# facebookresearch/KeypointNeRF

Measured on AMD Instinct MI355X. Metric: rendered rays/sec (64 coarse + 64 fine samples/ray), higher is better.
Workload: dtype f32 (dominant kernel: every fp32 operand as two fp16 pieces (22 bits, the residual formed exactly), three fp16-MFMA products per term set (hh hl lh: all terms above 2^-24 relative), fp32 accumulation; everything else fp32)

## Files before the change

### include/kpnerf.h

```cpp
#ifndef KPNERF_H
#define KPNERF_H

#include <stddef.h>
#include <stdint.h>

#ifdef __cplusplus
extern "C" {
#endif

#define KPN_ABI_VERSION 10
#define KPN_N_KPT 24
#define KPN_MAX_VIEWS 16

enum { KPN_OK = 0, KPN_EINVAL = -1, KPN_ELAUNCH = -2, KPN_EWORKSPACE = -3 };

int kpn_abi_version(void);
const char* kpn_last_error(void);
int kpn_is_device_build(void);

size_t kpn_plain_weight_floats(void);
size_t kpn_packed_weight_floats(void);
int kpn_pack_weights(const float* plain_host, float* packed_host);
int kpn_pack_weights_device(const float* plain_dev, float* packed_dev, void* stream);

typedef struct kpn_scene_desc {
    int32_t n_views;
    int32_t src_h, src_w;
    int32_t geo0_h, geo0_w;
    int32_t geo1_h, geo1_w;
    int32_t tex_h, tex_w;
    int32_t disable_fg_mask;
    float znear, zfar;
    float nml_scale;
    float sigma;
    const float* KRT;
    const float* extrin;
    const float* kpt3d;
    const float* img;
    const uint8_t* fg_mask;
    const float* geo0;
    const float* geo1;
    const float* tex;
} kpn_scene_desc;

size_t kpn_scene_workspace_bytes(const kpn_scene_desc* desc);
int kpn_scene_prepare(const kpn_scene_desc* desc, void* scene_ws, void* stream);


int kpn_ray_bbox_intersection(const float* bounds, const float* orig, const float* direct, int64_t n_rays,
                              float* near_out, float* far_out, uint8_t* hit_out, void* stream);

int kpn_make_rays(const float* K, const float* RT, float znear, float zfar, const float* bounds, int32_t x0,
                  int32_t y0, int32_t step, int32_t nx, int32_t ny, float* dirs, float* cam_pos, float* near_out,
                  float* far_out, void* stream);

int kpn_importance_sample(const float* contrib, const float* z, const float* u, int64_t n_rays, int32_t d_minus_2,
                          int32_t n_samples, float* samples_out, void* stream);

int kpn_rgba2out(const float* rgba, const float* z, int64_t n_rays, int32_t n_samples, float* color, float* depth,
                 float* alpha, float* contrib, float* sdf, void* stream);

int kpn_rgba2out_backward(const float* rgba, const float* z, int64_t n_rays, int32_t n_samples, const float* d_color,
                          const float* d_depth, const float* d_alpha, const float* d_sdf, float* d_rgba, void* stream);

size_t kpn_geo_rows_backward_workspace_bytes(int64_t n_points, int32_t n_views);
int kpn_geo_rows_backward(const kpn_scene_desc* desc, const void* scene_ws, const float* packed_weights, int64_t n_points,
                          const float* pts, uint32_t keep_mask, const float* d_x, float* d_plain, float* d_geo0,
                          float* d_geo1, void* workspace, size_t workspace_bytes, void* stream);

size_t kpn_query_backward_geometry_workspace_bytes(int64_t n_points, int32_t n_views);
int kpn_query_backward_geometry(const kpn_scene_desc* desc, const void* scene_ws, const float* packed_weights,
                                int64_t n_points, const float* pts, int32_t mode, uint32_t keep_mask, const float* noise,
                                float noise_std, const float* d_out, float* d_plain, float* d_geo0, float* d_geo1,
                                void* workspace, size_t workspace_bytes, void* stream);

size_t kpn_query_backward_workspace_bytes(int64_t n_points, int32_t n_views);
int kpn_query_backward(const kpn_scene_desc* desc, const void* scene_ws, const float* packed_weights, int64_t n_points,
                       const float* pts, const float* view, int32_t mode, uint32_t keep_mask, const float* noise,
                       float noise_std, const float* d_out, float* d_plain, float* d_geo0, float* d_geo1, float* d_tex,
// ... 223 lines not shown
```

### keypointnerf_amd/csrc/api_render.hip

```cpp
namespace {
struct RenderLayout { size_t cam_pos, dirs, nearv, farv, zc, zf, zn, src, rgba, rgba_c, rgba_n, contrib, color, depth, alpha, sdf, query, total; int64_t chunk; };
int64_t pick_chunk(const kpn_scene_desc* d, const kpn_render_args* a) {
    const int64_t R = (int64_t)a->nx * a->ny;
    int64_t c = a->chunk_rays;
    if (c <= 0) {
        const int64_t cmax = 262144;
        const int64_t npass = (R + cmax - 1) / cmax;
        c = ((R + npass - 1) / npass + 63) / 64 * 64;
    }
    return c < R ? c : R;
}
RenderLayout render_layout(const kpn_scene_desc* d, const kpn_render_args* a) {
    RenderLayout L;
    const int64_t R = (int64_t)a->nx * a->ny;
    const int64_t C = pick_chunk(d, a);
    const int64_t Sfull = a->n_coarse + (a->fine ? a->n_fine : 0);
    Carver c;
    L.chunk = C;
    L.cam_pos = c.take(64);
    L.dirs = c.take((size_t)R * 3 * 4);
    L.nearv = c.take((size_t)R * 4);
    L.farv = c.take((size_t)R * 4);
    L.zc = c.take((size_t)C * a->n_coarse * 4);
    L.zf = c.take((size_t)C * Sfull * 4);
// ... 38 lines not shown
}

__global__ void k_store_planar(int64_t r0, int64_t n, int64_t R, int C, const float* __restrict__ src, float* __restrict__ dst) {
    const int64_t i = (int64_t)blockIdx.x * blockDim.x + threadIdx.x;
    if (i >= n * C) return;
    const int64_t r = i / C;
    const int c = (int)(i - r * C);
    dst[(int64_t)c * R + r0 + r] = src[i];
}
__global__ void k_load_planar(int64_t r0, int64_t n, int64_t R, int C, const float* __restrict__ src, float* __restrict__ dst) {
    const int64_t i = (int64_t)blockIdx.x * blockDim.x + threadIdx.x;
    if (i >= n * C) return;
    const int64_t r = i / C;
    const int c = (int)(i - r * C);
    dst[i] = src ? src[(int64_t)c * R + r0 + r] : 0.0f;
}
struct PlanarChunk {
    void* stream; int64_t r0, n, R;
    void store(float* dst, const float* src, int C) const {
        if (dst) KPN_LAUNCH(k_store_planar, grid1d(n * C, 256), dim3(256), stream, r0, n, R, C, src, dst);
    }
    void load(float* dst, const float* src, int C) const {
        KPN_LAUNCH(k_load_planar, grid1d(n * C, 256), dim3(256), stream, r0, n, R, C, src, dst);
    }
};

extern "C" size_t kpn_render_workspace_bytes(const kpn_scene_desc* d, const kpn_render_args* a) {
    if (check_desc(d) != KPN_OK || check_render(a) != KPN_OK) return 0;
    return render_layout(d, a).total;
}

static void launch_fine_samples(void* stream, int64_t n, int Sc, int Sf, const float* zc, const float* contrib,
                                const float* u, float* zf, float* znew, int16_t* src) {
    const dim3 grid((unsigned)(n + 3 < 4 * 8192 ? (n + 3) / 4 : 8192));
    if (Sc <= 64 && Sf <= 64)
        KPN_LAUNCH(k_fine_samples_w<true>, grid, dim3(256), stream, n, Sc, Sf, zc, contrib, u, zf, znew, src);
    else
        KPN_LAUNCH(k_fine_samples_w<false>, grid, dim3(256), stream, n, Sc, Sf, zc, contrib, u, zf, znew, src);
}

static int render_impl(const kpn_scene_desc* d, const void* scene_ws, const float* wp, const kpn_render_args* a,
                       const kpn_train_args* t, void* ws, size_t ws_bytes, void* stream) {
    if (int e = check_desc(d)) return e;
    if (int e = check_render(a)) return e;
    KPN_REQUIRE(scene_ws && wp && ws, "null pointer");
    if (t) if (int e = check_train(d, a, t, false)) return e;
    const RenderLayout L = render_layout(d, a);
    if (ws_bytes < L.total) return fail(KPN_EWORKSPACE, "render workspace too small");
    char* base = static_cast<char*>(ws);
    auto F = [&](size_t off) { return reinterpret_cast<float*>(base + off); };
    kpn_scene_dev sc = scene_dev(d, scene_ws);
    const int64_t R = (int64_t)a->nx * a->ny;
    const int Sc = a->n_coarse, Sf = a->fine ? a->n_fine : 0, Sfull = Sc + Sf;
    KPN_LAUNCH(k_make_rays, grid1d(R, 256), dim3(256), stream, a->K, a->RT, a->znear, a->zfar, a->bounds, (int)a->x0, (int)a->y0,
               (int)a->step, (int)(a->step_y > 0 ? a->step_y : a->step), (int)a->nx, (int)a->ny, t ? (const int*)t->pix : (const int*)nullptr, F(L.dirs), F(L.cam_pos),
               F(L.nearv), F(L.farv));
    for (int64_t r0 = 0; r0 < R; r0 += L.chunk) {
        const int64_t n = (R - r0) < L.chunk ? (R - r0) : L.chunk;
        const float* dirs = F(L.dirs) + r0 * 3;
        const PlanarChunk pl{stream, r0, n, R};
        KPN_LAUNCH(k_coarse_z, grid1d(n * Sc, 256), dim3(256), stream, n, Sc, (const float*)(F(L.nearv) + r0),
                   (const float*)(F(L.farv) + r0), t ? t->u_coarse + r0 * Sc : (const float*)nullptr, F(L.zc));
        kpn_points ps{nullptr, nullptr, F(L.cam_pos), dirs, F(L.zc), Sc,
                      (t && t->rand_noise_std != 0.0f) ? t->noise_coarse + r0 * Sc : nullptr, t ? t->rand_noise_std : 0.0f};
        sc.keep = t ? t->keep_coarse : 0xFFFFFFFFu;
        const char* nr = getenv("KPN_NO_COARSE_REUSE");
        const bool no_reuse = nr && atoi(nr);
        const bool reuse = (t == nullptr) && a->fine && !no_reuse;
// ... 235 lines not shown
```

### keypointnerf_amd/csrc/api_scene.hip

```cpp
namespace {
struct SceneLayout { size_t table, rgbm, geo0, geo1, tex, flags, total; };
SceneLayout scene_layout(const kpn_scene_desc* d) {
    SceneLayout L;
    Carver c;
    L.table = c.take((size_t)d->n_views * KPN_TBL_STRIDE, 64);
    L.rgbm = c.take((size_t)d->n_views * d->src_h * d->src_w * 4, 64);
    L.geo0 = c.take((size_t)d->n_views * d->geo0_h * d->geo0_w * 64, 64);
    L.geo1 = c.take((size_t)d->n_views * d->geo1_h * d->geo1_w * 8, 64);
    L.tex = c.take((size_t)d->n_views * d->tex_h * d->tex_w * 8, 64);
    L.flags = c.take((size_t)KPN_SCENE_FLAG_FLOATS, 64);
    L.total = c.o;
    return L;
}
int check_desc(const kpn_scene_desc* d) {
    KPN_REQUIRE(d != nullptr, "scene desc is null");
    KPN_REQUIRE(d->n_views >= 1 && d->n_views <= KPN_MAX_VIEWS, "n_views out of range");
    KPN_REQUIRE(d->src_h > 1 && d->src_w > 1 && d->geo0_h > 1 && d->geo0_w > 1 && d->geo1_h > 1 && d->geo1_w > 1 &&
                d->tex_h > 1 && d->tex_w > 1, "map sizes must be > 1");
    KPN_REQUIRE(d->zfar > d->znear && d->nml_scale > 0.0f && d->sigma > 0.0f, "bad scalar parameters");
    KPN_REQUIRE(d->KRT && d->extrin && d->kpt3d && d->img && d->geo0 && d->geo1 && d->tex, "null scene tensor");
    KPN_REQUIRE(d->disable_fg_mask || d->fg_mask, "fg_mask is null");
    return KPN_OK;
}
kpn_scene_dev scene_dev(const kpn_scene_desc* d, const void* ws) {
    const SceneLayout L = scene_layout(d);
    const float* base = static_cast<const float*>(ws);
    kpn_scene_dev s;
    s.V = d->n_views; s.H = d->src_h; s.W = d->src_w;
    s.g0h = d->geo0_h; s.g0w = d->geo0_w; s.g1h = d->geo1_h; s.g1w = d->geo1_w; s.th = d->tex_h; s.tw = d->tex_w;
    s.disable_fg_mask = d->disable_fg_mask;
    s.znear = d->znear; s.zfar = d->zfar; s.nml_scale = d->nml_scale;
    s.two_sigma2 = (float)(2.0 * ((double)d->sigma * (double)d->sigma));
    s.keep = 0xFFFFFFFFu;
    s.table = base + L.table; s.rgbm = base + L.rgbm; s.geo0 = base + L.geo0; s.geo1 = base + L.geo1; s.tex = base + L.tex;
    s.flags = base + L.flags;
    return s;
}
}

extern "C" size_t kpn_scene_workspace_bytes(const kpn_scene_desc* d) {
    if (check_desc(d) != KPN_OK) return 0;
    return scene_layout(d).total * sizeof(float);
}

extern "C" int kpn_scene_prepare(const kpn_scene_desc* d, void* scene_ws, void* stream) {
    if (int e = check_desc(d)) return e;
    KPN_REQUIRE(scene_ws != nullptr, "scene workspace is null");
    const SceneLayout L = scene_layout(d);
    float* base = static_cast<float*>(scene_ws);
    const int V = d->n_views;
    float* flags = base + L.flags;
    KPN_LAUNCH(k_scene_table, dim3(1), dim3(64), stream, V, d->KRT, d->extrin, d->kpt3d, base + L.table, flags);
    const int64_t HW = (int64_t)d->src_h * d->src_w;
    KPN_LAUNCH(k_pack_rgbm, grid1d(V * HW, 256), dim3(256), stream, (int64_t)(V * HW), HW, d->img,
               d->disable_fg_mask ? (const uint8_t*)nullptr : d->fg_mask, base + L.rgbm, flags);
    const int64_t hw0 = (int64_t)d->geo0_h * d->geo0_w, hw1 = (int64_t)d->geo1_h * d->geo1_w, hwt = (int64_t)d->tex_h * d->tex_w;
    KPN_LAUNCH(k_nchw_to_nhwc, grid1d(V * hw0 * 64, 256), dim3(256), stream, (int64_t)(V * hw0 * 64), 64, hw0, d->geo0, base + L.geo0, flags);
    KPN_LAUNCH(k_nchw_to_nhwc, grid1d(V * hw1 * 8, 256), dim3(256), stream, (int64_t)(V * hw1 * 8), 8, hw1, d->geo1, base + L.geo1, flags);
    KPN_LAUNCH(k_nchw_to_nhwc, grid1d(V * hwt * 8, 256), dim3(256), stream, (int64_t)(V * hwt * 8), 8, hwt, d->tex, base + L.tex, flags);
    return check_launch("kpn_scene_prepare");
}

extern "C" int kpn_ray_bbox_intersection(const float* bounds, const float* orig, const float* direct, int64_t R,
                                         float* near_o, float* far_o, uint8_t* hit_o, void* stream) {
    KPN_REQUIRE(bounds && orig && direct && near_o && far_o && hit_o, "null pointer");
    KPN_REQUIRE(R >= 0, "negative ray count");
    if (R == 0) return KPN_OK;
    KPN_LAUNCH(k_ray_bbox, grid1d(R, 256), dim3(256), stream, R, bounds, orig, direct, near_o, far_o, hit_o);
    return check_launch("kpn_ray_bbox_intersection");
}

extern "C" int kpn_make_rays(const float* K, const float* RT, float znear, float zfar, const float* bounds, int32_t x0,
                             int32_t y0, int32_t step, int32_t nx, int32_t ny, float* dirs, float* cam_pos,
                             float* near_o, float* far_o, void* stream) {
    KPN_REQUIRE(K && RT && bounds && dirs && cam_pos && near_o && far_o, "null pointer");
    KPN_REQUIRE(nx > 0 && ny > 0 && step > 0, "bad pixel grid");
    KPN_LAUNCH(k_make_rays, grid1d((int64_t)nx * ny, 256), dim3(256), stream, K, RT, znear, zfar, bounds, (int)x0, (int)y0,
               (int)step, (int)step, (int)nx, (int)ny, (const int*)nullptr, dirs, cam_pos, near_o, far_o);
    return check_launch("kpn_make_rays");
}

extern "C" int kpn_importance_sample(const float* contrib, const float* z, const float* u, int64_t R, int32_t Dm2,
                                     int32_t n, float* out, void* stream) {
    KPN_REQUIRE(contrib && z && out, "null pointer");
    KPN_REQUIRE(Dm2 >= 1 && Dm2 + 1 <= KPN_IS_MAXD, "bin count out of range (<= 128)");
    KPN_REQUIRE(n >= 1 && R >= 0, "bad sizes");
    if (R == 0) return KPN_OK;
    KPN_LAUNCH(k_importance, grid1d(R, 64), dim3(64), stream, R, (int)Dm2, (int)n, contrib, z, u, out);
    return check_launch("kpn_importance_sample");
}

static void launch_rgba2out(void* stream, int64_t R, int S, const float* rgba, const float* z, float* color, float* depth,
// ... 39 lines not shown
```

### keypointnerf_amd/csrc/ray_kernels.hip

```cpp
#include "kpn_device.h"

__device__ __forceinline__ void kpn_note_absmax(float* __restrict__ flags, float a) {
    int u = __float_as_int(a) & 0x7fffffff;
#pragma unroll
    for (int o = 32; o > 0; o >>= 1) { const int w = __shfl_xor(u, o); u = w > u ? w : u; }
    int* f = reinterpret_cast<int*>(flags);
    if ((threadIdx.x & 63) == 0 && u > *reinterpret_cast<volatile int*>(f)) atomicMax(f, u);
}
__device__ __forceinline__ float kpn_absmax2(float a, float b) {
    const int x = __float_as_int(a) & 0x7fffffff, y = __float_as_int(b) & 0x7fffffff;
    return __int_as_float(x > y ? x : y);
}

__global__ void k_scene_table(int V, const float* __restrict__ KRT, const float* __restrict__ extrin,
                              const float* __restrict__ kpt3d, float* __restrict__ table, float* __restrict__ flags) {
    const int v = blockIdx.x * blockDim.x + threadIdx.x;
    if (v < KPN_SCENE_FLAG_FLOATS) flags[v] = 0.0f;
    if (v >= V) return;
    float* tb = table + (size_t)v * KPN_TBL_STRIDE;
    const float* M = KRT + v * 16;
    const float* E = extrin + v * 16;
    for (int i = 0; i < 12; ++i) { tb[KPN_TBL_KRT + i] = M[i]; tb[KPN_TBL_EXT + i] = E[i]; }
    double a[4][8];
    for (int i = 0; i < 4; ++i)
        for (int j = 0; j < 4; ++j) { a[i][j] = (double)M[i * 4 + j]; a[i][4 + j] = (i == j) ? 1.0 : 0.0; }
    for (int c = 0; c < 4; ++c) {
        int p = c;
        for (int r = c + 1; r < 4; ++r) if (fabs(a[r][c]) > fabs(a[p][c])) p = r;
        if (p != c) for (int j = 0; j < 8; ++j) { double t = a[c][j]; a[c][j] = a[p][j]; a[p][j] = t; }
        const double d = a[c][c];
        for (int j = 0; j < 8; ++j) a[c][j] /= d;
        for (int r = 0; r < 4; ++r) if (r != c) {
            const double f = a[r][c];
            for (int j = 0; j < 8; ++j) a[r][j] -= f * a[c][j];
        }
    }
    for (int i = 0; i < 3; ++i) tb[KPN_TBL_CPOS + i] = (float)a[i][7];
    tb[KPN_TBL_CPOS + 3] = 0.0f;
    for (int k = 0; k < KPN_NKPT; ++k)
        for (int i = 0; i < 3; ++i)
            tb[KPN_TBL_KCAM + k * 3 + i] =
                KADD(kpn_dot3(kpt3d[k * 3 + 0], kpt3d[k * 3 + 1], kpt3d[k * 3 + 2], E[i * 4 + 0], E[i * 4 + 1], E[i * 4 + 2]),
                     E[i * 4 + 3]);
    for (int i = KPN_TBL_KCAM + KPN_NKPT * 3; i < KPN_TBL_STRIDE; ++i) tb[i] = 0.0f;
}

__global__ void k_pack_rgbm(int64_t npix_total, int64_t HW, const float* __restrict__ img,
                            const uint8_t* __restrict__ mask, float* __restrict__ out, float* __restrict__ flags) {
    const int64_t i = (int64_t)blockIdx.x * blockDim.x + threadIdx.x;
    float amax = 0.0f;
    if (i < npix_total) {
        const int64_t v = i / HW, p = i - v * HW;
        float4 o;
        o.x = img[(v * 3 + 0) * HW + p];
        o.y = img[(v * 3 + 1) * HW + p];
        o.z = img[(v * 3 + 2) * HW + p];
        o.w = mask ? (mask[i] ? 1.0f : 0.0f) : 1.0f;
        reinterpret_cast<float4*>(out)[i] = o;
        amax = kpn_absmax2(kpn_absmax2(o.x, o.y), o.z);
    }
    kpn_note_absmax(flags, amax);
}

__global__ void k_nchw_to_nhwc(int64_t total, int C, int64_t hw, const float* __restrict__ in, float* __restrict__ out,
                               float* __restrict__ flags) {
    const int64_t i = (int64_t)blockIdx.x * blockDim.x + threadIdx.x;
    float x = 0.0f;
    if (i < total) {
        const int c = (int)(i % C);
        const int64_t vp = i / C;
        const int64_t v = vp / hw, p = vp - v * hw;
        x = in[(v * C + c) * hw + p];
        out[i] = x;
    }
    kpn_note_absmax(flags, x);
}

__device__ __forceinline__ void kpn_ray_aabb(const float* __restrict__ bounds, float ox, float oy, float oz, float dx,
                                             float dy, float dz, float& near_o, float& far_o, int& hit) {
    float bmin[3], bmax[3], o[3] = {ox, oy, oz}, d[3] = {dx, dy, dz};
#pragma unroll
    for (int i = 0; i < 3; ++i) {
        bmin[i] = KADD(bounds[i], -0.01f);
        bmax[i] = KADD(bounds[3 + i], 0.01f);
        if (fabsf(d[i]) < 1e-5f) d[i] = 1e-5f;
    }
    int cnt = 0;
    float pint[2][3];
    const float eps = 1e-6f;
#pragma unroll
    for (int s = 0; s < 6; ++s) {
        const int ax = s % 3;
        const float bound = (s < 3) ? bmin[ax] : bmax[ax];
        const float t = KSUB(bound, o[ax]) / d[ax];
        const float p0 = KADD(KMUL(t, d[0]), o[0]), p1 = KADD(KMUL(t, d[1]), o[1]), p2 = KADD(KMUL(t, d[2]), o[2]);
        const int inside = (p0 >= KSUB(bmin[0], eps)) && (p0 <= KADD(bmax[0], eps)) && (p1 >= KSUB(bmin[1], eps)) &&
                           (p1 <= KADD(bmax[1], eps)) && (p2 >= KSUB(bmin[2], eps)) && (p2 <= KADD(bmax[2], eps));
        if (inside) {
            if (cnt < 2) { pint[cnt][0] = p0; pint[cnt][1] = p1; pint[cnt][2] = p2; }
            ++cnt;
        }
    }
    if (cnt == 2) {
        const float nr = sqrtf(kpn_dot3(d[0], d[1], d[2], d[0], d[1], d[2]));
        float dd[2];
#pragma unroll
        for (int k = 0; k < 2; ++k) {
            const float e0 = KSUB(pint[k][0], o[0]), e1 = KSUB(pint[k][1], o[1]), e2 = KSUB(pint[k][2], o[2]);
// ... 297 lines not shown
                                                   const float* __restrict__ zin, const float* __restrict__ u,
                                                   float* __restrict__ out) {
    __shared__ float cdf_s[64][KPN_IS_MAXD];
    const int t = threadIdx.x;
    const int64_t r = (int64_t)blockIdx.x * 64 + t;
    if (r >= R) return;
    const int C = Dm2 + 1;
    const float* c = contrib + r * Dm2;
    const float* zz = zin + r * C;
    float sum = 0.0f;
    for (int i = 0; i < Dm2; ++i) sum = KADD(sum, KADD(c[i], 1e-5f));
    float run = 0.0f;
    cdf_s[t][0] = 0.0f;
    for (int i = 0; i < Dm2; ++i) {
        run = KADD(run, KADD(c[i], 1e-5f) / sum);
        cdf_s[t][i + 1] = run;
    }
    for (int k = 0; k < n; ++k) {
        const float s = u ? u[r * n + k] : kpn_linspace01(k, n);
        int lo = 0, hi = C;
        while (lo < hi) {
            const int mid = (lo + hi) >> 1;
            if (cdf_s[t][mid] <= s) lo = mid + 1; else hi = mid;
        }
        const int ip = lo - 1 < 0 ? 0 : lo - 1;
        const int in = lo > C - 1 ? C - 1 : lo;
        const float num = KSUB(s, cdf_s[t][ip]);
        float den = KSUB(cdf_s[t][in], cdf_s[t][ip]);
        if (den < 1e-5f) den = 1.0f;
        out[r * n + k] = KADD(zz[ip], KMUL(num / den, KSUB(zz[in], zz[ip])));
    }
}

#ifndef KPN_SIMT_EMU
#define KPN_READLANE_F(v, i) __int_as_float(__builtin_amdgcn_readlane(__float_as_int(v), (i)))
#else
#define KPN_READLANE_F(v, i) __shfl((v), (i))
#endif
template <bool SMALL>
__global__ __launch_bounds__(256) void k_fine_samples_w(int64_t R, int Sc, int Sf, const float* __restrict__ zc,
                                                        const float* __restrict__ contrib, const float* __restrict__ u,
                                                        float* __restrict__ zf, float* __restrict__ znew,
                                                        int16_t* __restrict__ src) {
    constexpr int NE = SMALL ? 1 : 2;
    constexpr int W = 64 * NE;
    __shared__ float q_s[SMALL ? 1 : 4][SMALL ? 1 : W];
    __shared__ float cdf_s[4][W + 1];
    __shared__ float zn_s[4][W];
    __shared__ float ev_s[4][2 * W];
    const int lane = threadIdx.x & 63, w = threadIdx.x >> 6;
    const int Dm2 = Sc - 2, C = Sc - 1, Sfull = Sc + Sf;
    for (int64_t r = (int64_t)blockIdx.x * 4 + w; r < R; r += (int64_t)gridDim.x * 4) {
        const float* c = contrib + r * Sc + 1;
        const float* z = zc + r * Sc;
        for (int i = lane; i < Sc; i += 64) ev_s[w][i] = z[i];
        if constexpr (SMALL) {
            float q = lane < Dm2 ? KADD(c[lane], 1e-5f) : 0.0f;
            float sum = 0.0f;
            for (int i = 0; i < Dm2; ++i) sum = KADD(sum, KPN_READLANE_F(q, i));
            q = q / sum;
            float run = 0.0f, mine = 0.0f;
            for (int i = 0; i < Dm2; ++i) {
                run = KADD(run, KPN_READLANE_F(q, i));
                mine = lane == i + 1 ? run : mine;
            }
            if (lane < C) cdf_s[w][lane] = mine;
        } else {
            for (int i = lane; i < Dm2; i += 64) q_s[w][i] = KADD(c[i], 1e-5f);
            KPN_WAVE_SYNC();
            float sum = 0.0f;
            if (lane == 0)
                for (int i = 0; i < Dm2; ++i) sum = KADD(sum, q_s[w][i]);
            sum = __shfl(sum, 0);
            for (int i = lane; i < Dm2; i += 64) q_s[w][i] = q_s[w][i] / sum;
            KPN_WAVE_SYNC();
            if (lane == 0) {
                float run = 0.0f;
                cdf_s[w][0] = 0.0f;
                for (int i = 0; i < Dm2; ++i) { run = KADD(run, q_s[w][i]); cdf_s[w][i + 1] = run; }
            }
        }
        KPN_WAVE_SYNC();
        float v[NE];
        for (int e = 0; e < NE; ++e) {
            const int k = lane + 64 * e;
            v[e] = 0.0f;
            if (k < Sf) {
                const float sv = u ? u[r * Sf + k] : kpn_linspace01(k, Sf);
                int lo = 0, hi = C;
                while (lo < hi) {
                    const int mid = (lo + hi) >> 1;
                    if (cdf_s[w][mid] <= sv) lo = mid + 1; else hi = mid;
                }
                const int ip = lo - 1 < 0 ? 0 : lo - 1;
                const int in = lo > C - 1 ? C - 1 : lo;
                const float num = KSUB(sv, cdf_s[w][ip]);
                float den = KSUB(cdf_s[w][in], cdf_s[w][ip]);
                if (den < 1e-5f) den = 1.0f;
                const float zp = KMUL(0.5f, KADD(ev_s[w][ip + 1], ev_s[w][ip]));
                const float zq = KMUL(0.5f, KADD(ev_s[w][in + 1], ev_s[w][in]));
                v[e] = KADD(zp, KMUL(num / den, KSUB(zq, zp)));
                zn_s[w][k] = v[e];
            }
        }
        KPN_WAVE_SYNC();
        int rk[NE];
        int unsorted = 0;
        for (int e = 0; e < NE; ++e) {
            const int k = lane + 64 * e;
            rk[e] = k;
            unsorted |= (k + 1 < Sf) && !(v[e] <= zn_s[w][k + 1 < W ? k + 1 : k]);
        }
        if (__any(unsorted)) {
            for (int e = 0; e < NE; ++e) rk[e] = 0;
            for (int j = 0; j < Sf; ++j) {
                const float o = zn_s[w][j];
                for (int e = 0; e < NE; ++e) rk[e] += (o < v[e]) || (o == v[e] && j < lane + 64 * e);
            }
        }
        for (int e = 0; e < NE; ++e)
            if (lane + 64 * e < Sf) ev_s[w][Sc + rk[e]] = v[e];
        KPN_WAVE_SYNC();
        if (znew)
            for (int k = lane; k < Sf; k += 64) znew[r * Sf + k] = ev_s[w][Sc + k];
        int csorted = 1;
        for (int i = lane; i + 1 < Sc; i += 64) csorted &= ev_s[w][i] <= ev_s[w][i + 1];
        if (__all(csorted)) {
            for (int i = lane; i < Sc; i += 64) {
                const float a = ev_s[w][i];
                int lo = 0, hi = Sf;
                while (lo < hi) { const int mid = (lo + hi) >> 1; if (ev_s[w][Sc + mid] < a) lo = mid + 1; else hi = mid; }
                zf[r * Sfull + i + lo] = a;
                if (src) src[r * Sfull + i + lo] = (int16_t)i;
            }
            for (int k = lane; k < Sf; k += 64) {
                const float b = ev_s[w][Sc + k];
                int lo = 0, hi = Sc;
                while (lo < hi) { const int mid = (lo + hi) >> 1; if (ev_s[w][mid] <= b) lo = mid + 1; else hi = mid; }
                zf[r * Sfull + k + lo] = b;
                if (src) src[r * Sfull + k + lo] = (int16_t)(Sc + k);
            }
        } else {
            for (int id = lane; id < Sfull; id += 64) {
                const float a = ev_s[w][id];
                int rank = 0;
                for (int j = 0; j < Sfull; ++j) { const float o = ev_s[w][j]; rank += (o < a) || (o == a && j < id); }
                zf[r * Sfull + rank] = a;
                if (src) src[r * Sfull + rank] = (int16_t)id;
            }
        }
        KPN_WAVE_SYNC();
    }
}

__global__ void k_frame_to_rgb8(int HW, int bgr, const float* __restrict__ chw, uint8_t* __restrict__ hwc) {
    const int i = blockIdx.x * blockDim.x + threadIdx.x;
    if (i >= HW) return;
#pragma unroll
    for (int c = 0; c < 3; ++c) {
        const float v = fminf(fmaxf(chw[(size_t)c * HW + i], 0.0f), 1.0f);
        hwc[(size_t)i * 3 + (bgr ? 2 - c : c)] = (uint8_t)(int)KMUL(v, 255.0f);
    }
}

__global__ __launch_bounds__(256) void k_mse_psnr(int64_t n, const float* __restrict__ a, const float* __restrict__ b,
                                                  double* __restrict__ partial, int* __restrict__ ticket,
                                                  double* __restrict__ out2) {
    __shared__ double red[1][256];
    double acc[1] = {0.0};
    for (int64_t i = (int64_t)blockIdx.x * blockDim.x + threadIdx.x; i < n; i += (int64_t)gridDim.x * blockDim.x) {
        const float d = KSUB(a[i], b[i]);
        acc[0] += (double)KMUL(d, d);
    }
    if (kpn_block_sums_last(acc, red, partial, ticket, blockIdx.x, gridDim.x, threadIdx.x == 0)) {
        const double tot = kpn_partials_in_order(partial, gridDim.x, 1, 0);
        const double mse = tot / (double)n;
        out2[0] = mse;
        out2[1] = -10.0 * log(mse) / log(10.0);
    }
}

__global__ __launch_bounds__(256) void k_ssim_vertical(const float* __restrict__ pred, const float* __restrict__ gt, int H, int W,
                                                       int x0, int y0, int w, int h, float* __restrict__ tmp) {
    const int64_t i = (int64_t)blockIdx.x * blockDim.x + threadIdx.x;
// ... 45 lines not shown
```

### keypointnerf_amd/lib.py

```python
import ctypes
import os

import torch

_HERE = os.path.dirname(os.path.abspath(__file__))
DEFAULT_LIB = os.path.join(_HERE, "_lib", "libkpnerf_hip.so")

c_f = ctypes.c_float
c_i32 = ctypes.c_int32
c_i64 = ctypes.c_int64
c_p = ctypes.c_void_p
c_sz = ctypes.c_size_t


class SceneDesc(ctypes.Structure):
    _fields_ = [(n, c_i32) for n in ("n_views", "src_h", "src_w", "geo0_h", "geo0_w", "geo1_h", "geo1_w", "tex_h",
                                     "tex_w", "disable_fg_mask")] + \
               [(n, c_f) for n in ("znear", "zfar", "nml_scale", "sigma")] + \
               [(n, c_p) for n in ("KRT", "extrin", "kpt3d", "img", "fg_mask", "geo0", "geo1", "tex")]


class RenderStages(ctypes.Structure):
    _fields_ = [(n, c_p) for n in ("z_coarse", "rgba_coarse", "z_fine", "rgba_fine", "dirs", "cam_pos")]

# ... 25 lines not shown


class AdamSegment(ctypes.Structure):
    _fields_ = [(n, c_p) for n in ("param", "grad", "exp_avg", "exp_avg_sq")] + [("count", c_i64)]


class AdamArgs(ctypes.Structure):
    _fields_ = [("segments_host", ctypes.POINTER(AdamSegment)), ("n_segments", c_i32), ("step", c_i64)] + \
               [(n, ctypes.c_double) for n in ("lr", "beta1", "beta2", "eps", "weight_decay")]


class Conv2dDesc(ctypes.Structure):
    _fields_ = [(n, c_i32) for n in ("N", "H", "W", "cin", "cout", "k", "pad", "has_bias")]


class GroupNormDesc(ctypes.Structure):
    _fields_ = [(n, c_i32) for n in ("N", "H", "W", "C", "G", "affine", "relu")] + [("eps", c_f)]


class ResampleDesc(ctypes.Structure):
    _fields_ = [(n, c_i32) for n in ("N", "h", "w", "C")]


_SIGNATURES = {
    "kpn_abi_version": (ctypes.c_int, []),
    "kpn_last_error": (ctypes.c_char_p, []),
    "kpn_is_device_build": (ctypes.c_int, []),
    "kpn_plain_weight_floats": (c_sz, []),
    "kpn_packed_weight_floats": (c_sz, []),
    "kpn_pack_weights": (ctypes.c_int, [c_p, c_p]),
    "kpn_pack_weights_device": (ctypes.c_int, [c_p, c_p, c_p]),
    "kpn_scene_workspace_bytes": (c_sz, [ctypes.POINTER(SceneDesc)]),
    "kpn_scene_prepare": (ctypes.c_int, [ctypes.POINTER(SceneDesc), c_p, c_p]),
    "kpn_ray_bbox_intersection": (ctypes.c_int, [c_p, c_p, c_p, c_i64, c_p, c_p, c_p, c_p]),
    "kpn_make_rays": (ctypes.c_int, [c_p, c_p, c_f, c_f, c_p, c_i32, c_i32, c_i32, c_i32, c_i32, c_p, c_p, c_p, c_p, c_p]),
    "kpn_importance_sample": (ctypes.c_int, [c_p, c_p, c_p, c_i64, c_i32, c_i32, c_p, c_p]),
    "kpn_rgba2out": (ctypes.c_int, [c_p, c_p, c_i64, c_i32, c_p, c_p, c_p, c_p, c_p, c_p]),
    "kpn_rgba2out_backward": (ctypes.c_int, [c_p, c_p, c_i64, c_i32, c_p, c_p, c_p, c_p, c_p, c_p]),
    "kpn_geo_rows_backward_workspace_bytes": (c_sz, [c_i64, c_i32]),
    "kpn_geo_rows_backward": (ctypes.c_int, [ctypes.POINTER(SceneDesc), c_p, c_p, c_i64, c_p, ctypes.c_uint32, c_p, c_p, c_p,
                                             c_p, c_p, c_sz, c_p]),
    "kpn_query_backward_geometry_workspace_bytes": (c_sz, [c_i64, c_i32]),
    "kpn_query_backward_geometry": (ctypes.c_int, [ctypes.POINTER(SceneDesc), c_p, c_p, c_i64, c_p, c_i32, ctypes.c_uint32, c_p,
                                                   ctypes.c_float, c_p, c_p, c_p, c_p, c_p, c_sz, c_p]),
    "kpn_query_backward_workspace_bytes": (c_sz, [c_i64, c_i32]),
    "kpn_query_backward": (ctypes.c_int, [ctypes.POINTER(SceneDesc), c_p, c_p, c_i64, c_p, c_p, c_i32, ctypes.c_uint32, c_p,
                                          ctypes.c_float, c_p, c_p, c_p, c_p, c_p, c_p, c_sz, c_p]),
    "kpn_render_rays_train_backward_workspace_bytes": (c_sz, [ctypes.POINTER(SceneDesc), ctypes.POINTER(RenderArgs)]),
    "kpn_render_rays_train_backward": (ctypes.c_int, [ctypes.POINTER(SceneDesc), c_p, c_p, ctypes.POINTER(RenderArgs),
                                                      ctypes.POINTER(TrainArgs), ctypes.POINTER(RenderGrads), c_p, c_p, c_p, c_p,
                                                      c_p, c_sz, c_p]),
    "kpn_set_geo_rows_mode": (ctypes.c_int, [c_i32]),
    "kpn_get_geo_rows_mode": (ctypes.c_int, []),
    "kpn_packed_f16_range_check": (ctypes.c_int, [c_p, c_p, c_p]),
    "kpn_set_fuse_mode": (ctypes.c_int, [c_i32]),
    "kpn_get_fuse_mode": (ctypes.c_int, []),
    "kpn_set_density_first": (ctypes.c_int, [c_i32]),
    "kpn_get_density_first": (ctypes.c_int, []),
    "kpn_density_stats": (ctypes.c_int, [c_p, c_p, c_p, c_i32]),
    "kpn_density_first_passes": (ctypes.c_int, [c_p, c_p, c_i32]),
    "kpn_bwd_profile_enable": (ctypes.c_int, [c_i32]),
    "kpn_bwd_profile_collect": (ctypes.c_int, [c_p, c_p, c_p, c_p, c_p]),
    "kpn_set_range_guard": (ctypes.c_int, [c_i32]),
    "kpn_get_range_guard": (ctypes.c_int, []),
    "kpn_range_guard_count": (ctypes.c_int, [c_p, c_p]),
    "kpn_ssim_scratch_bytes": (c_sz, [c_i32, c_i32]),
# ... 110 lines not shown
```

Measured before the change: 12.47 million.

## Tile scene-prep transposes, parallelize scene table, batch fine-sample CDF rows per wave

Scene preparation now uses tiled NCHW-to-NHWC transposes through shared memory with optional float4 loads, block-level absmax reduction before the atomic, a per-view parallel table build, and a tiled RGB+mask pack. The fine importance-sampling kernel now processes groups of rays per wave, loading contrib rows into shared memory and building each row's CDF in one lane, in place of the readlane-based wave scan. A scene-layout query API and int32 size checks are also added. These target global memory coalescing and per-ray serial overheads, at the cost of more shared memory and serial per-lane CDF loops.

```diff
diff --git a/include/kpnerf.h b/include/kpnerf.h
--- a/include/kpnerf.h
+++ b/include/kpnerf.h
@@ -45,6 +45,7 @@
 
 size_t kpn_scene_workspace_bytes(const kpn_scene_desc* desc);
 int kpn_scene_prepare(const kpn_scene_desc* desc, void* scene_ws, void* stream);
+int kpn_scene_layout(const kpn_scene_desc* desc, size_t offsets[6]);
 
 
 int kpn_ray_bbox_intersection(const float* bounds, const float* orig, const float* direct, int64_t n_rays,
diff --git a/keypointnerf_amd/csrc/api_render.hip b/keypointnerf_amd/csrc/api_render.hip
--- a/keypointnerf_amd/csrc/api_render.hip
+++ b/keypointnerf_amd/csrc/api_render.hip
@@ -94,8 +94,10 @@
 
 static void launch_fine_samples(void* stream, int64_t n, int Sc, int Sf, const float* zc, const float* contrib,
                                 const float* u, float* zf, float* znew, int16_t* src) {
-    const dim3 grid((unsigned)(n + 3 < 4 * 8192 ? (n + 3) / 4 : 8192));
-    if (Sc <= 64 && Sf <= 64)
+    const bool small = Sc <= 64 && Sf <= 64;
+    const int64_t per = 4 * KPN_FINE_GROUP(small);
+    const dim3 grid((unsigned)((n + per - 1) / per < 8192 ? (n + per - 1) / per : 8192));
+    if (small)
         KPN_LAUNCH(k_fine_samples_w<true>, grid, dim3(256), stream, n, Sc, Sf, zc, contrib, u, zf, znew, src);
     else
         KPN_LAUNCH(k_fine_samples_w<false>, grid, dim3(256), stream, n, Sc, Sf, zc, contrib, u, zf, znew, src);
diff --git a/keypointnerf_amd/csrc/api_scene.hip b/keypointnerf_amd/csrc/api_scene.hip
--- a/keypointnerf_amd/csrc/api_scene.hip
+++ b/keypointnerf_amd/csrc/api_scene.hip
@@ -17,6 +17,8 @@
     KPN_REQUIRE(d->n_views >= 1 && d->n_views <= KPN_MAX_VIEWS, "n_views out of range");
     KPN_REQUIRE(d->src_h > 1 && d->src_w > 1 && d->geo0_h > 1 && d->geo0_w > 1 && d->geo1_h > 1 && d->geo1_w > 1 &&
                 d->tex_h > 1 && d->tex_w > 1, "map sizes must be > 1");
+    KPN_REQUIRE((int64_t)d->src_h * d->src_w <= INT32_MAX && (int64_t)d->geo0_h * d->geo0_w <= INT32_MAX &&
+                (int64_t)d->geo1_h * d->geo1_w <= INT32_MAX && (int64_t)d->tex_h * d->tex_w <= INT32_MAX, "map too large");
     KPN_REQUIRE(d->zfar > d->znear && d->nml_scale > 0.0f && d->sigma > 0.0f, "bad scalar parameters");
     KPN_REQUIRE(d->KRT && d->extrin && d->kpt3d && d->img && d->geo0 && d->geo1 && d->tex, "null scene tensor");
     KPN_REQUIRE(d->disable_fg_mask || d->fg_mask, "fg_mask is null");
@@ -43,6 +45,14 @@
     return scene_layout(d).total * sizeof(float);
 }
 
+extern "C" int kpn_scene_layout(const kpn_scene_desc* d, size_t offsets[6]) {
+    if (int e = check_desc(d)) return e;
+    KPN_REQUIRE(offsets != nullptr, "offsets is null");
+    const SceneLayout L = scene_layout(d);
+    offsets[0] = L.table; offsets[1] = L.rgbm; offsets[2] = L.geo0; offsets[3] = L.geo1; offsets[4] = L.tex; offsets[5] = L.flags;
+    return KPN_OK;
+}
+
 extern "C" int kpn_scene_prepare(const kpn_scene_desc* d, void* scene_ws, void* stream) {
     if (int e = check_desc(d)) return e;
     KPN_REQUIRE(scene_ws != nullptr, "scene workspace is null");
@@ -50,14 +60,18 @@
     float* base = static_cast<float*>(scene_ws);
     const int V = d->n_views;
     float* flags = base + L.flags;
-    KPN_LAUNCH(k_scene_table, dim3(1), dim3(64), stream, V, d->KRT, d->extrin, d->kpt3d, base + L.table, flags);
-    const int64_t HW = (int64_t)d->src_h * d->src_w;
-    KPN_LAUNCH(k_pack_rgbm, grid1d(V * HW, 256), dim3(256), stream, (int64_t)(V * HW), HW, d->img,
+    KPN_LAUNCH(k_scene_table, dim3(V), dim3(128), stream, V, d->KRT, d->extrin, d->kpt3d, base + L.table, flags);
+    const int HW = d->src_h * d->src_w;
+    const int ptiles = (HW + KPN_PACK_PIX - 1) / KPN_PACK_PIX;
+    KPN_LAUNCH(k_pack_rgbm, dim3(V * ptiles), dim3(256), stream, HW, ptiles, d->img,
                d->disable_fg_mask ? (const uint8_t*)nullptr : d->fg_mask, base + L.rgbm, flags);
-    const int64_t hw0 = (int64_t)d->geo0_h * d->geo0_w, hw1 = (int64_t)d->geo1_h * d->geo1_w, hwt = (int64_t)d->tex_h * d->tex_w;
-    KPN_LAUNCH(k_nchw_to_nhwc, grid1d(V * hw0 * 64, 256), dim3(256), stream, (int64_t)(V * hw0 * 64), 64, hw0, d->geo0, base + L.geo0, flags);
-    KPN_LAUNCH(k_nchw_to_nhwc, grid1d(V * hw1 * 8, 256), dim3(256), stream, (int64_t)(V * hw1 * 8), 8, hw1, d->geo1, base + L.geo1, flags);
-    KPN_LAUNCH(k_nchw_to_nhwc, grid1d(V * hwt * 8, 256), dim3(256), stream, (int64_t)(V * hwt * 8), 8, hwt, d->tex, base + L.tex, flags);
+    auto vec = [](const float* p, int hw) { return (hw % 4 == 0 && reinterpret_cast<uintptr_t>(p) % 16 == 0) ? 1 : 0; };
+    const int hw0 = d->geo0_h * d->geo0_w, hw1 = d->geo1_h * d->geo1_w, hwt = d->tex_h * d->tex_w;
+    const int t0 = (hw0 + KPN_NHWC_TILE / 64 - 1) / (KPN_NHWC_TILE / 64), t1 = (hw1 + KPN_NHWC_TILE / 8 - 1) / (KPN_NHWC_TILE / 8),
+              tt = (hwt + KPN_NHWC_TILE / 8 - 1) / (KPN_NHWC_TILE / 8);
+    KPN_LAUNCH(k_nchw_to_nhwc<64>, dim3(V * t0), dim3(256), stream, hw0, t0, vec(d->geo0, hw0), d->geo0, base + L.geo0, flags);
+    KPN_LAUNCH(k_nchw_to_nhwc<8>, dim3(V * t1), dim3(256), stream, hw1, t1, vec(d->geo1, hw1), d->geo1, base + L.geo1, flags);
+    KPN_LAUNCH(k_nchw_to_nhwc<8>, dim3(V * tt), dim3(256), stream, hwt, tt, vec(d->tex, hwt), d->tex, base + L.tex, flags);
     return check_launch("kpn_scene_prepare");
 }
 
diff --git a/keypointnerf_amd/csrc/ray_kernels.hip b/keypointnerf_amd/csrc/ray_kernels.hip
--- a/keypointnerf_amd/csrc/ray_kernels.hip
+++ b/keypointnerf_amd/csrc/ray_kernels.hip
@@ -1,79 +1,125 @@
 #include "kpn_device.h"
 
-__device__ __forceinline__ void kpn_note_absmax(float* __restrict__ flags, float a) {
-    int u = __float_as_int(a) & 0x7fffffff;
-#pragma unroll
-    for (int o = 32; o > 0; o >>= 1) { const int w = __shfl_xor(u, o); u = w > u ? w : u; }
-    int* f = reinterpret_cast<int*>(flags);
-    if ((threadIdx.x & 63) == 0 && u > *reinterpret_cast<volatile int*>(f)) atomicMax(f, u);
-}
-__device__ __forceinline__ float kpn_absmax2(float a, float b) {
-    const int x = __float_as_int(a) & 0x7fffffff, y = __float_as_int(b) & 0x7fffffff;
-    return __int_as_float(x > y ? x : y);
-}
-
-__global__ void k_scene_table(int V, const float* __restrict__ KRT, const float* __restrict__ extrin,
-                              const float* __restrict__ kpt3d, float* __restrict__ table, float* __restrict__ flags) {
-    const int v = blockIdx.x * blockDim.x + threadIdx.x;
-    if (v < KPN_SCENE_FLAG_FLOATS) flags[v] = 0.0f;
-    if (v >= V) return;
+__device__ __forceinline__ int kpn_abs_bits(float a) { return __float_as_int(a) & 0x7fffffff; }
+__device__ __forceinline__ int kpn_abs_bits4(int u, const float4& x) {
+    const int a = max(kpn_abs_bits(x.x), kpn_abs_bits(x.y)), b = max(kpn_abs_bits(x.z), kpn_abs_bits(x.w));
+    return max(u, max(a, b));
+}
+__device__ __forceinline__ void kpn_note_absmax(float* __restrict__ flags, int u) {
+    __shared__ int wmax_s[4];
+#pragma unroll
+    for (int o = 32; o > 0; o >>= 1) u = max(u, __shfl_xor(u, o));
+    if ((threadIdx.x & 63) == 0) wmax_s[threadIdx.x >> 6] = u;
+    __syncthreads();
+    if (threadIdx.x == 0) {
+        u = max(max(wmax_s[0], wmax_s[1]), max(wmax_s[2], wmax_s[3]));
+        int* f = reinterpret_cast<int*>(flags);
+        if (u > *reinterpret_cast<volatile int*>(f)) atomicMax(f, u);
+    }
+}
+
+__global__ __launch_bounds__(128) void k_scene_table(int V, const float* __restrict__ KRT, const float* __restrict__ extrin,
+                                                     const float* __restrict__ kpt3d, float* __restrict__ table,
+                                                     float* __restrict__ flags) {
+    const int v = blockIdx.x, t = threadIdx.x;
+    if (v == 0 && t < KPN_SCENE_FLAG_FLOATS) flags[t] = 0.0f;
     float* tb = table + (size_t)v * KPN_TBL_STRIDE;
     const float* M = KRT + v * 16;
     const float* E = extrin + v * 16;
-    for (int i = 0; i < 12; ++i) { tb[KPN_TBL_KRT + i] = M[i]; tb[KPN_TBL_EXT + i] = E[i]; }
-    double a[4][8];
-    for (int i = 0; i < 4; ++i)
-        for (int j = 0; j < 4; ++j) { a[i][j] = (double)M[i * 4 + j]; a[i][4 + j] = (i == j) ? 1.0 : 0.0; }
-    for (int c = 0; c < 4; ++c) {
-        int p = c;
-        for (int r = c + 1; r < 4; ++r) if (fabs(a[r][c]) > fabs(a[p][c])) p = r;
-        if (p != c) for (int j = 0; j < 8; ++j) { double t = a[c][j]; a[c][j] = a[p][j]; a[p][j] = t; }
-        const double d = a[c][c];
-        for (int j = 0; j < 8; ++j) a[c][j] /= d;
-        for (int r = 0; r < 4; ++r) if (r != c) {
-            const double f = a[r][c];
-            for (int j = 0; j < 8; ++j) a[r][j] -= f * a[c][j];
-        }
-    }
-    for (int i = 0; i < 3; ++i) tb[KPN_TBL_CPOS + i] = (float)a[i][7];
-    tb[KPN_TBL_CPOS + 3] = 0.0f;
-    for (int k = 0; k < KPN_NKPT; ++k)
-        for (int i = 0; i < 3; ++i)
-            tb[KPN_TBL_KCAM + k * 3 + i] =
-                KADD(kpn_dot3(kpt3d[k * 3 + 0], kpt3d[k * 3 + 1], kpt3d[k * 3 + 2], E[i * 4 + 0], E[i * 4 + 1], E[i * 4 + 2]),
-                     E[i * 4 + 3]);
-    for (int i = KPN_TBL_KCAM + KPN_NKPT * 3; i < KPN_TBL_STRIDE; ++i) tb[i] = 0.0f;
-}
-
-__global__ void k_pack_rgbm(int64_t npix_total, int64_t HW, const float* __restrict__ img,
-                            const uint8_t* __restrict__ mask, float* __restrict__ out, float* __restrict__ flags) {
-    const int64_t i = (int64_t)blockIdx.x * blockDim.x + threadIdx.x;
-    float amax = 0.0f;
-    if (i < npix_total) {
-        const int64_t v = i / HW, p = i - v * HW;
-        float4 o;
-        o.x = img[(v * 3 + 0) * HW + p];
-        o.y = img[(v * 3 + 1) * HW + p];
-        o.z = img[(v * 3 + 2) * HW + p];
-        o.w = mask ? (mask[i] ? 1.0f : 0.0f) : 1.0f;
-        reinterpret_cast<float4*>(out)[i] = o;
-        amax = kpn_absmax2(kpn_absmax2(o.x, o.y), o.z);
+    if (t == 64) {
+        double a[4][8];
+        for (int i = 0; i < 4; ++i)
+            for (int j = 0; j < 4; ++j) { a[i][j] = (double)M[i * 4 + j]; a[i][4 + j] = (i == j) ? 1.0 : 0.0; }
+        for (int c = 0; c < 4; ++c) {
+            int p = c;
+            for (int r = c + 1; r < 4; ++r) if (fabs(a[r][c]) > fabs(a[p][c])) p = r;
+            if (p != c) for (int j = 0; j < 8; ++j) { double s = a[c][j]; a[c][j] = a[p][j]; a[p][j] = s; }
+            const double d = a[c][c];
+            for (int j = 0; j < 8; ++j) a[c][j] /= d;
+            for (int r = 0; r < 4; ++r) if (r != c) {
+                const double f = a[r][c];
+                for (int j = 0; j < 8; ++j) a[r][j] -= f * a[c][j];
+            }
+        }
+        for (int i = 0; i < 3; ++i) tb[KPN_TBL_CPOS + i] = (float)a[i][7];
+        tb[KPN_TBL_CPOS + 3] = 0.0f;
+    }
+    if (t >= 64) return;
+    if (t < 12) { tb[KPN_TBL_KRT + t] = M[t]; tb[KPN_TBL_EXT + t] = E[t]; }
+    for (int e = t; e < KPN_NKPT * 3; e += 64) {
+        const int k = e / 3, i = e - k * 3;
+        tb[KPN_TBL_KCAM + e] =
+            KADD(kpn_dot3(kpt3d[k * 3 + 0], kpt3d[k * 3 + 1], kpt3d[k * 3 + 2], E[i * 4 + 0], E[i * 4 + 1], E[i * 4 + 2]),
+                 E[i * 4 + 3]);
+    }
+    for (int i = KPN_TBL_KCAM + KPN_NKPT * 3 + t; i < KPN_TBL_STRIDE; i += 64) tb[i] = 0.0f;
+}
+
+#define KPN_PACK_PIX 1024
+__global__ __launch_bounds__(256) void k_pack_rgbm(int HW, int tiles, const float* __restrict__ img,
+                                                   const uint8_t* __restrict__ mask, float* __restrict__ out,
+                                                   float* __restrict__ flags) {
+    const int v = blockIdx.x / tiles;
+    const int p0 = (blockIdx.x - v * tiles) * KPN_PACK_PIX + (threadIdx.x >> 6) * 256 + (threadIdx.x & 63);
+    const float* src = img + (size_t)v * 3 * HW;
+    const uint8_t* m = mask ? mask + (size_t)v * HW : nullptr;
+    float4* dst = reinterpret_cast<float4*>(out) + (size_t)v * HW;
+    int amax = 0;
+#pragma unroll
+    for (int j = 0; j < 4; ++j) {
+        const int p = p0 + 64 * j;
+        if (p < HW) {
+            float4 o;
+            o.x = src[p];
+            o.y = src[(size_t)HW + p];
+            o.z = src[2 * (size_t)HW + p];
+            o.w = m ? (m[p] ? 1.0f : 0.0f) : 1.0f;
+            dst[p] = o;
+            amax = max(amax, max(max(kpn_abs_bits(o.x), kpn_abs_bits(o.y)), kpn_abs_bits(o.z)));
+        }
     }
     kpn_note_absmax(flags, amax);
 }
 
-__global__ void k_nchw_to_nhwc(int64_t total, int C, int64_t hw, const float* __restrict__ in, float* __restrict__ out,
-                               float* __restrict__ flags) {
-    const int64_t i = (int64_t)blockIdx.x * blockDim.x + threadIdx.x;
-    float x = 0.0f;
-    if (i < total) {
-        const int c = (int)(i % C);
-        const int64_t vp = i / C;
-        const int64_t v = vp / hw, p = vp - v * hw;
-        x = in[(v * C + c) * hw + p];
-        out[i] = x;
-    }
-    kpn_note_absmax(flags, x);
+#define KPN_NHWC_TILE 4096
+template <int C>
+__global__ __launch_bounds__(256) void k_nchw_to_nhwc(int hw, int tiles, int vec, const float* __restrict__ in,
+                                                      float* __restrict__ out, float* __restrict__ flags) {
+    constexpr int TP = KPN_NHWC_TILE / C, PITCH = TP + 1;
+    __shared__ float tile_s[C * PITCH];
+    const int v = blockIdx.x / tiles;
+    const int p0 = (blockIdx.x - v * tiles) * TP;
+    const int np = hw - p0 < TP ? hw - p0 : TP;
+    const float* src = in + (size_t)v * C * hw + p0;
+    int amax = 0;
+    if (vec) {
+        for (int e = threadIdx.x; e < C * (TP / 4); e += 256) {
+            const int c = e / (TP / 4), p = (e % (TP / 4)) * 4;
+            if (p < np) {
+                const float4 x = *reinterpret_cast<const float4*>(src + (size_t)c * hw + p);
+                float* d = tile_s + c * PITCH + p;
+                d[0] = x.x; d[1] = x.y; d[2] = x.z; d[3] = x.w;
+                amax = kpn_abs_bits4(amax, x);
+            }
+        }
+    } else {
+        for (int e = threadIdx.x; e < C * TP; e += 256) {
+            const int c = e / TP, p = e % TP;
+            if (p < np) {
+                const float x = src[(size_t)c * hw + p];
+                tile_s[c * PITCH + p] = x;
+                amax = max(amax, kpn_abs_bits(x));
+            }
+        }
+    }
+    __syncthreads();
+    float4* dst = reinterpret_cast<float4*>(out + ((size_t)v * hw + p0) * C);
+    for (int o4 = threadIdx.x; o4 < np * (C / 4); o4 += 256) {
+        const int p = o4 / (C / 4), c = (o4 % (C / 4)) * 4;
+        const float* t = tile_s + c * PITCH + p;
+        dst[o4] = make_float4(t[0], t[PITCH], t[2 * PITCH], t[3 * PITCH]);
+    }
+    kpn_note_absmax(flags, amax);
 }
 
 __device__ __forceinline__ void kpn_ray_aabb(const float* __restrict__ bounds, float ox, float oy, float oz, float dx,
@@ -437,11 +483,7 @@
     }
 }
 
-#ifndef KPN_SIMT_EMU
-#define KPN_READLANE_F(v, i) __int_as_float(__builtin_amdgcn_readlane(__float_as_int(v), (i)))
-#else
-#define KPN_READLANE_F(v, i) __shfl((v), (i))
-#endif
+#define KPN_FINE_GROUP(SMALL) ((SMALL) ? 16 : 8)
 template <bool SMALL>
 __global__ __launch_bounds__(256) void k_fine_samples_w(int64_t R, int Sc, int Sf, const float* __restrict__ zc,
                                                         const float* __restrict__ contrib, const float* __restrict__ u,
@@ -449,112 +491,109 @@
                                                         int16_t* __restrict__ src) {
     constexpr int NE = SMALL ? 1 : 2;
     constexpr int W = 64 * NE;
-    __shared__ float q_s[SMALL ? 1 : 4][SMALL ? 1 : W];
-    __shared__ float cdf_s[4][W + 1];
+    constexpr int G = KPN_FINE_GROUP(SMALL);
+    __shared__ float row_s[4][G][W + 1];
     __shared__ float zn_s[4][W];
     __shared__ float ev_s[4][2 * W];
     const int lane = threadIdx.x & 63, w = threadIdx.x >> 6;
     const int Dm2 = Sc - 2, C = Sc - 1, Sfull = Sc + Sf;
-    for (int64_t r = (int64_t)blockIdx.x * 4 + w; r < R; r += (int64_t)gridDim.x * 4) {
-        const float* c = contrib + r * Sc + 1;
-        const float* z = zc + r * Sc;
-        for (int i = lane; i < Sc; i += 64) ev_s[w][i] = z[i];
-        if constexpr (SMALL) {
-            float q = lane < Dm2 ? KADD(c[lane], 1e-5f) : 0.0f;
+    for (int64_t r0 = ((int64_t)blockIdx.x * 4 + w) * G; r0 < R; r0 += (int64_t)gridDim.x * 4 * G) {
+        const int ng = R - r0 < G ? (int)(R - r0) : G;
+        float zr[NE];
+        for (int e = 0; e < NE; ++e) zr[e] = lane + 64 * e < Sc ? zc[r0 * Sc + lane + 64 * e] : 0.0f;
+        for (int g = 0; g < ng; ++g)
+            for (int i = lane; i < Sc; i += 64) row_s[w][g][i] = contrib[(r0 + g) * Sc + i];
+        KPN_WAVE_SYNC();
+        if (lane < ng) {
+            float* q = row_s[w][lane];
             float sum = 0.0f;
-            for (int i = 0; i < Dm2; ++i) sum = KADD(sum, KPN_READLANE_F(q, i));
-            q = q / sum;
-            float run = 0.0f, mine = 0.0f;
+            for (int i = 0; i < Dm2; ++i) sum = KADD(sum, KADD(q[i + 1], 1e-5f));
+            float run = 0.0f;
+            q[0] = 0.0f;
             for (int i = 0; i < Dm2; ++i) {
-                run = KADD(run, KPN_READLANE_F(q, i));
-                mine = lane == i + 1 ? run : mine;
-            }
-            if (lane < C) cdf_s[w][lane] = mine;
-        } else {
-            for (int i = lane; i < Dm2; i += 64) q_s[w][i] = KADD(c[i], 1e-5f);
+                run = KADD(run, KADD(q[i + 1], 1e-5f) / sum);
+                q[i + 1] = run;
+            }
+        }
+        KPN_WAVE_SYNC();
+        for (int g = 0; g < ng; ++g) {
+            const int64_t r = r0 + g;
+            const float* cdf = row_s[w][g];
+            for (int e = 0; e < NE; ++e)
+                if (lane + 64 * e < Sc) ev_s[w][lane + 64 * e] = zr[e];
+            if (g + 1 < ng)
+                for (int e = 0; e < NE; ++e) zr[e] = lane + 64 * e < Sc ? zc[(r + 1) * Sc + lane + 64 * e] : 0.0f;
             KPN_WAVE_SYNC();
-            float sum = 0.0f;
-            if (lane == 0)
-                for (int i = 0; i < Dm2; ++i) sum = KADD(sum, q_s[w][i]);
-            sum = __shfl(sum, 0);
-            for (int i = lane; i < Dm2; i += 64) q_s[w][i] = q_s[w][i] / sum;
+            float v[NE];
+            for (int e = 0; e < NE; ++e) {
+                const int k = lane + 64 * e;
+                v[e] = 0.0f;
+                if (k < Sf) {
+                    const float sv = u ? u[r * Sf + k] : kpn_linspace01(k, Sf);
+                    int lo = 0, hi = C;
+                    while (lo < hi) {
+                        const int mid = (lo + hi) >> 1;
+                        if (cdf[mid] <= sv) lo = mid + 1; else hi = mid;
+                    }
+                    const int ip = lo - 1 < 0 ? 0 : lo - 1;
+                    const int in = lo > C - 1 ? C - 1 : lo;
+                    const float num = KSUB(sv, cdf[ip]);
+                    float den = KSUB(cdf[in], cdf[ip]);
+                    if (den < 1e-5f) den = 1.0f;
+                    const float zp = KMUL(0.5f, KADD(ev_s[w][ip + 1], ev_s[w][ip]));
+                    const float zq = KMUL(0.5f, KADD(ev_s[w][in + 1], ev_s[w][in]));
+                    v[e] = KADD(zp, KMUL(num / den, KSUB(zq, zp)));
+                    zn_s[w][k] = v[e];
+                }
+            }
             KPN_WAVE_SYNC();
-            if (lane == 0) {
-                float run = 0.0f;
-                cdf_s[w][0] = 0.0f;
-                for (int i = 0; i < Dm2; ++i) { run = KADD(run, q_s[w][i]); cdf_s[w][i + 1] = run; }
-            }
-        }
-        KPN_WAVE_SYNC();
-        float v[NE];
-        for (int e = 0; e < NE; ++e) {
-            const int k = lane + 64 * e;
-            v[e] = 0.0f;
-            if (k < Sf) {
-                const float sv = u ? u[r * Sf + k] : kpn_linspace01(k, Sf);
-                int lo = 0, hi = C;
-                while (lo < hi) {
-                    const int mid = (lo + hi) >> 1;
-                    if (cdf_s[w][mid] <= sv) lo = mid + 1; else hi = mid;
+            int rk[NE];
+            int unsorted = 0;
+            for (int e = 0; e < NE; ++e) {
+                const int k = lane + 64 * e;
+                rk[e] = k;
+                unsorted |= (k + 1 < Sf) && !(v[e] <= zn_s[w][k + 1 < W ? k + 1 : k]);
+            }
+            if (__any(unsorted)) {
+                for (int e = 0; e < NE; ++e) rk[e] = 0;
+                for (int j = 0; j < Sf; ++j) {
+                    const float o = zn_s[w][j];
+                    for (int e = 0; e < NE; ++e) rk[e] += (o < v[e]) || (o == v[e] && j < lane + 64 * e);
                 }
-                const int ip = lo - 1 < 0 ? 0 : lo - 1;
-                const int in = lo > C - 1 ? C - 1 : lo;
-                const float num = KSUB(sv, cdf_s[w][ip]);
-                float den = KSUB(cdf_s[w][in], cdf_s[w][ip]);
-                if (den < 1e-5f) den = 1.0f;
-                const float zp = KMUL(0.5f, KADD(ev_s[w][ip + 1], ev_s[w][ip]));
-                const float zq = KMUL(0.5f, KADD(ev_s[w][in + 1], ev_s[w][in]));
-                v[e] = KADD(zp, KMUL(num / den, KSUB(zq, zp)));
-                zn_s[w][k] = v[e];
-            }
-        }
-        KPN_WAVE_SYNC();
-        int rk[NE];
-        int unsorted = 0;
-        for (int e = 0; e < NE; ++e) {
-            const int k = lane + 64 * e;
-            rk[e] = k;
-            unsorted |= (k + 1 < Sf) && !(v[e] <= zn_s[w][k + 1 < W ? k + 1 : k]);
-        }
-        if (__any(unsorted)) {
-            for (int e = 0; e < NE; ++e) rk[e] = 0;
-            for (int j = 0; j < Sf; ++j) {
-                const float o = zn_s[w][j];
-                for (int e = 0; e < NE; ++e) rk[e] += (o < v[e]) || (o == v[e] && j < lane + 64 * e);
-            }
-        }
-        for (int e = 0; e < NE; ++e)
-            if (lane + 64 * e < Sf) ev_s[w][Sc + rk[e]] = v[e];
-        KPN_WAVE_SYNC();
-        if (znew)
-            for (int k = lane; k < Sf; k += 64) znew[r * Sf + k] = ev_s[w][Sc + k];
-        int csorted = 1;
-        for (int i = lane; i + 1 < Sc; i += 64) csorted &= ev_s[w][i] <= ev_s[w][i + 1];
-        if (__all(csorted)) {
-            for (int i = lane; i < Sc; i += 64) {
-                const float a = ev_s[w][i];
-                int lo = 0, hi = Sf;
-                while (lo < hi) { const int mid = (lo + hi) >> 1; if (ev_s[w][Sc + mid] < a) lo = mid + 1; else hi = mid; }
-                zf[r * Sfull + i + lo] = a;
-                if (src) src[r * Sfull + i + lo] = (int16_t)i;
-            }
-            for (int k = lane; k < Sf; k += 64) {
-                const float b = ev_s[w][Sc + k];
-                int lo = 0, hi = Sc;
-                while (lo < hi) { const int mid = (lo + hi) >> 1; if (ev_s[w][mid] <= b) lo = mid + 1; else hi = mid; }
-                zf[r * Sfull + k + lo] = b;
-                if (src) src[r * Sfull + k + lo] = (int16_t)(Sc + k);
-            }
-        } else {
-            for (int id = lane; id < Sfull; id += 64) {
-                const float a = ev_s[w][id];
-                int rank = 0;
-                for (int j = 0; j < Sfull; ++j) { const float o = ev_s[w][j]; rank += (o < a) || (o == a && j < id); }
-                zf[r * Sfull + rank] = a;
-                if (src) src[r * Sfull + rank] = (int16_t)id;
-            }
-        }
-        KPN_WAVE_SYNC();
+            }
+            for (int e = 0; e < NE; ++e)
+                if (lane + 64 * e < Sf) ev_s[w][Sc + rk[e]] = v[e];
+            KPN_WAVE_SYNC();
+            if (znew)
+                for (int k = lane; k < Sf; k += 64) znew[r * Sf + k] = ev_s[w][Sc + k];
+            int csorted = 1;
+            for (int i = lane; i + 1 < Sc; i += 64) csorted &= ev_s[w][i] <= ev_s[w][i + 1];
+            if (__all(csorted)) {
+                for (int i = lane; i < Sc; i += 64) {
+                    const float a = ev_s[w][i];
+                    int lo = 0, hi = Sf;
+                    while (lo < hi) { const int mid = (lo + hi) >> 1; if (ev_s[w][Sc + mid] < a) lo = mid + 1; else hi = mid; }
+                    zf[r * Sfull + i + lo] = a;
+                    if (src) src[r * Sfull + i + lo] = (int16_t)i;
+                }
+                for (int k = lane; k < Sf; k += 64) {
+                    const float b = ev_s[w][Sc + k];
+                    int lo = 0, hi = Sc;
+                    while (lo < hi) { const int mid = (lo + hi) >> 1; if (ev_s[w][mid] <= b) lo = mid + 1; else hi = mid; }
+                    zf[r * Sfull + k + lo] = b;
+                    if (src) src[r * Sfull + k + lo] = (int16_t)(Sc + k);
+                }
+            } else {
+                for (int id = lane; id < Sfull; id += 64) {
+                    const float a = ev_s[w][id];
+                    int rank = 0;
+                    for (int j = 0; j < Sfull; ++j) { const float o = ev_s[w][j]; rank += (o < a) || (o == a && j < id); }
+                    zf[r * Sfull + rank] = a;
+                    if (src) src[r * Sfull + rank] = (int16_t)id;
+                }
+            }
+            KPN_WAVE_SYNC();
+        }
     }
 }
 
diff --git a/keypointnerf_amd/lib.py b/keypointnerf_amd/lib.py
--- a/keypointnerf_amd/lib.py
+++ b/keypointnerf_amd/lib.py
@@ -81,6 +81,7 @@
     "kpn_pack_weights_device": (ctypes.c_int, [c_p, c_p, c_p]),
     "kpn_scene_workspace_bytes": (c_sz, [ctypes.POINTER(SceneDesc)]),
     "kpn_scene_prepare": (ctypes.c_int, [ctypes.POINTER(SceneDesc), c_p, c_p]),
+    "kpn_scene_layout": (ctypes.c_int, [ctypes.POINTER(SceneDesc), ctypes.POINTER(c_sz)]),
     "kpn_ray_bbox_intersection": (ctypes.c_int, [c_p, c_p, c_p, c_i64, c_p, c_p, c_p, c_p]),
     "kpn_make_rays": (ctypes.c_int, [c_p, c_p, c_f, c_f, c_p, c_i32, c_i32, c_i32, c_i32, c_i32, c_p, c_p, c_p, c_p, c_p]),
     "kpn_importance_sample": (ctypes.c_int, [c_p, c_p, c_p, c_i64, c_i32, c_i32, c_p, c_p]),
```

New measurement: 12.84 million (median of 6 runs). 1.03x the previous value.
